# shubhamchandak94/HARC

Hardware: AMD Instinct MI355X
Metric: Mreads/s reorder+encode, 100 bp (higher is better)
Workload: dtype u64 (2-bit packed bases, XOR+popcount)

## Files before the change

### harc_amd/csrc/prims.hip

```cpp
#include "devutil.h"
#include <rocprim/rocprim.hpp>

int harc_tmp_reserve(harc_amd_ctx *c, size_t bytes)
{
    if (bytes <= c->tmp_bytes) return HARC_AMD_OK;
    if (c->d_tmp) harc_raw_free(c, c->d_tmp);
    c->d_tmp = nullptr; c->tmp_bytes = 0;
    size_t want = bytes + (bytes >> 3) + 4096;
    RC_TRY(harc_raw_alloc(c, &c->d_tmp, want));
    c->tmp_bytes = want;
    return HARC_AMD_OK;
}

#define PRIM_CALL(call_with_tmp)                                \
    do {                                                        \
        size_t bytes = 0; void *tmp = nullptr;                  \
        HIP_TRY(call_with_tmp);                                 \
        RC_TRY(harc_tmp_reserve(c, bytes));                     \
        tmp = c->d_tmp; bytes = c->tmp_bytes;                   \
        HIP_TRY(call_with_tmp);                                 \
    } while (0)

int prim_sort_pairs_u64_u32(harc_amd_ctx *c, const uint64_t *kin, uint64_t *kout, const uint32_t *vin, uint32_t *vout, size_t n, unsigned end_bit)
{
// ... 96 lines not shown
                M = __shfl(v, 63, 64);
            } else if (v > M) M = v;
            C += (uint32_t)__popcll(hb);
        }
    }
    if (!WRITE) {
        for (int o = 32; o > 0; o >>= 1) { const long long x = __shfl_xor(M, o, 64); if (x > M) M = x; }
        if (lane == 0) part[w] = BinPart{ M, C, 0u };
    }
}
int prim_bins_scan(harc_amd_ctx *c, const uint64_t *skeys, size_t n, uint64_t cap, uint32_t *binstart, uint64_t *q, uint32_t *nbins, void *scratch, size_t scratch_bytes)
{
    if (n == 0) return HARC_AMD_OK;
    const size_t room = scratch_bytes / (2 * sizeof(BinPart));
    if (room == 0 || n > 0xFFFFFFFFull || (n + room - 1) / room > (1u << 30) || room > 0x7FFFFFFFull) { harc_set_error("prim_bins_scan: %zu keys, scratch of %zu bytes", n, scratch_bytes); return HARC_AMD_EINVAL; }
    size_t seg = (n + room - 1) / room;
    if (seg < BINS_SEG_MIN) seg = BINS_SEG_MIN;
    seg = (seg + 64 * BINS_UNROLL - 1) / (64 * BINS_UNROLL) * (64 * BINS_UNROLL);
    const uint32_t nseg = (uint32_t)((n + seg - 1) / seg);
    BinPart *part = (BinPart *)scratch, *front = part + nseg;
    const dim3 grid((nseg + 3) / 4);
    hipLaunchKernelGGL(k_bins_pass<false>, grid, dim3(256), 0, c->stream, skeys, (uint32_t)n, cap, (uint32_t)seg, nseg, part, (uint32_t *)nullptr, (uint64_t *)nullptr, (uint32_t *)nullptr);
    PRIM_CALL(rocprim::exclusive_scan(tmp, bytes, part, front, BinPart{ BINS_NONE, 0u, 0u }, (size_t)nseg, BinPartOp(), c->stream));
    hipLaunchKernelGGL(k_bins_pass<true>, grid, dim3(256), 0, c->stream, skeys, (uint32_t)n, cap, (uint32_t)seg, nseg, front, binstart, q, nbins);
    HIP_TRY(hipGetLastError());
    return HARC_AMD_OK;
}

struct ContigPart { uint64_t s; uint32_t c, last; };
struct ContigPartOp {
    __host__ __device__ ContigPart operator()(const ContigPart &a, const ContigPart &b) const { return ContigPart{ a.s + b.s, a.c + b.c, a.last > b.last ? a.last : b.last }; }
};
#define CONTIG_SEG_MIN 2048u
#define CONTIG_SEGS 16384u
#define CONTIG_UNROLL 4
template <bool WRITE> __global__ __launch_bounds__(256) void k_contig_pass(const uint8_t *flag, const uint8_t *pos, uint32_t n, uint32_t L, uint32_t q, uint32_t cut, uint32_t seg, uint32_t nseg,
                                                                         ContigPart *part, uint8_t *head, uint32_t *cid, uint64_t *gstart, uint32_t *chead, unsigned long long *info)
{
    const uint32_t w = (blockIdx.x * 256u + threadIdx.x) >> 6;
    if (w >= nseg) return;
    const uint32_t lane = threadIdx.x & 63;
    const unsigned long long upto = ~0ull >> (63 - lane);
    uint32_t C = 0, last = 0; uint64_t G = 0;
    if (WRITE) { C = part[w].c; last = part[w].last; G = part[w].s; }
    const uint64_t base = (uint64_t)w * seg, end = base + seg < n ? base + seg : (uint64_t)n;
    uint32_t rem = (uint32_t)(base % q);
    for (uint64_t at = base; at < end; at += 64u * CONTIG_UNROLL) {
        uint8_t f[CONTIG_UNROLL], p[CONTIG_UNROLL];
#pragma unroll
        for (int u = 0; u < CONTIG_UNROLL; u++) { const uint64_t i = at + 64u * u + lane; f[u] = i < end ? flag[i] : (uint8_t)0; p[u] = i < end ? pos[i] : (uint8_t)0; }
#pragma unroll
        for (int u = 0; u < CONTIG_UNROLL; u++) {
            const uint64_t i0 = at + 64u * u, i = i0 + lane;
            const uint32_t m = rem + lane;
            const bool sh = q >= 128u ? (m == 0 || m == q) : (m % q) == 0;
            if (q >= 128u) { rem += 64u; if (rem >= q) rem -= q; } else rem = (rem + 64u) % q;
            const bool h = i < end && (f[u] == '0' || sh);
            const unsigned long long hb = __ballot(h);
            uint32_t v = i >= end ? 0u : h ? (i == 0 ? 0u : L) : (uint32_t)p[u];
            if (WRITE) {
                const uint32_t rank = C + (uint32_t)__popcll(hb & upto) - (h ? 1u : 0u);
                for (int d = 1; d < 64; d <<= 1) { const uint32_t o = __shfl_up(v, d, 64); if (lane >= (uint32_t)d) v += o; }
                const uint64_t g = G + v;
                const unsigned long long mine = hb & upto;
                const uint32_t l1 = mine ? (uint32_t)i0 + 63u - (uint32_t)__clzll(mine) : last;
                if (i < end) {
                    head[i] = h ? 1 : 0; cid[i] = rank; gstart[i] = g;
                    if (h) chead[rank] = (uint32_t)i;
                    if (sh) info[3 + (uint32_t)i / q] = g;
                    if ((uint32_t)i - l1 > cut) info[2] = 1;
                    if (i + 1 == n) { info[0] = rank + (h ? 1u : 0u); info[1] = g + L; }
                }
                G += __shfl(v, 63, 64);
            } else {
                for (int o = 32; o > 0; o >>= 1) v += __shfl_xor(v, o, 64);
                G += v;
            }
            if (hb) last = (uint32_t)i0 + 63u - (uint32_t)__clzll(hb);
            C += (uint32_t)__popcll(hb);
        }
    }
    if (!WRITE && lane == 0) part[w] = ContigPart{ G, C, last };
}
int prim_contig_scan(harc_amd_ctx *c, const uint8_t *flag, const uint8_t *pos, size_t n, uint32_t L, uint32_t q, uint32_t cut, uint8_t *head, uint32_t *cid, uint64_t *gstart,
                     uint32_t *chead, unsigned long long *info)
{
    if (n == 0) return HARC_AMD_OK;
    if (n > 0xFFFFFFFFull || q == 0) { harc_set_error("prim_contig_scan: %zu reads, shards of %u", n, q); return HARC_AMD_EINVAL; }
    size_t seg = (n + CONTIG_SEGS - 1) / CONTIG_SEGS;
    if (seg < CONTIG_SEG_MIN) seg = CONTIG_SEG_MIN;
    seg = (seg + 64 * CONTIG_UNROLL - 1) / (64 * CONTIG_UNROLL) * (64 * CONTIG_UNROLL);
    const uint32_t nseg = (uint32_t)((n + seg - 1) / seg);
    PoolScope scope(c);
    ContigPart *part = nullptr; RC_TRY(dalloc(c, &part, (size_t)2 * nseg));
    ContigPart *front = part + nseg;
    const dim3 grid((nseg + 3) / 4);
    HIP_TRY(hipMemsetAsync(info + 2, 0, 8, c->stream));
    hipLaunchKernelGGL(k_contig_pass<false>, grid, dim3(256), 0, c->stream, flag, pos, (uint32_t)n, L, q, cut, (uint32_t)seg, nseg, part, (uint8_t *)nullptr, (uint32_t *)nullptr, (uint64_t *)nullptr,
                       (uint32_t *)nullptr, (unsigned long long *)nullptr);
    PRIM_CALL(rocprim::exclusive_scan(tmp, bytes, part, front, ContigPart{ 0, 0u, 0u }, (size_t)nseg, ContigPartOp(), c->stream));
    hipLaunchKernelGGL(k_contig_pass<true>, grid, dim3(256), 0, c->stream, flag, pos, (uint32_t)n, L, q, cut, (uint32_t)seg, nseg, front, head, cid, gstart, chead, info);
    HIP_TRY(hipGetLastError());
    return HARC_AMD_OK;
}

__global__ void k_selftest_grid(uint64_t n, unsigned long long *out)
{
    const uint64_t i = harc_gid();
    unsigned long long one = i < n ? 1ULL : 0ULL, idx = i < n ? (unsigned long long)i : 0ULL;
    for (int o = 32; o > 0; o >>= 1) { one += __shfl_xor(one, o, 64); idx += __shfl_xor(idx, o, 64); }
    if ((threadIdx.x & 63) == 0 && one) { atomicAdd(&out[0], one); atomicAdd(&out[1], idx); }
}
__global__ void k_selftest_grid32(uint32_t n, unsigned long long *out)
{
    const uint32_t i = harc_gid32();
    unsigned long long one = i < n ? 1ULL : 0ULL, idx = i < n ? (unsigned long long)i : 0ULL;
    for (int o = 32; o > 0; o >>= 1) { one += __shfl_xor(one, o, 64); idx += __shfl_xor(idx, o, 64); }
    if ((threadIdx.x & 63) == 0 && one) { atomicAdd(&out[0], one); atomicAdd(&out[1], idx); }
}
__global__ void k_selftest_fold(uint64_t n, unsigned long long *out)
{
    const uint64_t wave = harc_bid() * 4 + (threadIdx.x >> 6);
    const int lane = threadIdx.x & 63;
    const uint64_t i = wave * 16 + (uint64_t)(lane >> 2);
    const bool mine = i < n && (lane & 3) == 0;
    unsigned long long one = mine ? 1ULL : 0ULL, idx = mine ? (unsigned long long)i : 0ULL;
    for (int o = 32; o > 0; o >>= 1) { one += __shfl_xor(one, o, 64); idx += __shfl_xor(idx, o, 64); }
    if (lane == 0 && one) { atomicAdd(&out[0], one); atomicAdd(&out[1], idx); }
}
extern "C" int harc_amd_selftest_launch(harc_amd_ctx *c, uint64_t n, uint64_t *visited, uint64_t *index_sum)
{
    if (!c || !visited || !index_sum) return HARC_AMD_EINVAL;
    HIP_TRY(hipSetDevice(c->P.device));
    unsigned long long *d = nullptr, h[6] = { 0, 0, 0, 0, 0, 0 };
    HIP_TRY(hipMalloc((void **)&d, sizeof h));
    const bool n32 = n <= 0xFFFFFFFFull;
    hipError_t e = hipMemsetAsync(d, 0, sizeof h, c->stream);
    if (e == hipSuccess) { hipLaunchKernelGGL(k_selftest_grid, harc_grid256(n), dim3(256), 0, c->stream, n, d); e = hipGetLastError(); }
    if (e == hipSuccess && n32) { hipLaunchKernelGGL(k_selftest_grid32, harc_grid256(n), dim3(256), 0, c->stream, (uint32_t)n, d + 2); e = hipGetLastError(); }
    if (e == hipSuccess) { hipLaunchKernelGGL(k_selftest_fold, harc_fold256((n + 63) / 64), dim3(256), 0, c->stream, n, d + 4); e = hipGetLastError(); }
    if (e == hipSuccess) e = hipMemcpyAsync(h, d, sizeof h, hipMemcpyDeviceToHost, c->stream);
    if (e == hipSuccess) e = hipStreamSynchronize(c->stream);
    (void)hipFree(d);
    if (e != hipSuccess) { harc_set_error("harc_amd_selftest_launch: %s", hipGetErrorString(e)); return HARC_AMD_ENODEVICE; }
    int k = 0;
    if (n32 && (h[2] != h[0] || h[3] != h[1])) k = 2;
    else if (h[4] != h[0] || h[5] != h[1]) k = 4;
    if (k) harc_set_error("harc_amd_selftest_launch: %s visited %llu items (index sum %llx), the thread-per-item grid %llu (%llx)", k == 2 ? "harc_gid32" : "harc_fold256 / harc_bid", h[k], h[k + 1], h[0], h[1]);
    *visited = h[k]; *index_sum = h[k + 1];
    return k ? HARC_AMD_EINTERNAL : HARC_AMD_OK;
}
```

### harc_amd/csrc/stage2.hip

```cpp
#include "devutil.h"
#include <time.h>
#include <algorithm>
#include <stdlib.h>

#define TUPLE_NONE 0xFFFFFFFFFFFFFFFFULL

struct S2Args {
    int L, W, W3, thresh_s, maxsearch;
    int ds[2], de[2], kbits[2];
    uint32_t M, S, T, q, nC;
    uint64_t total;
    const uint64_t *oreads;
    const uint64_t *reads;
    uint64_t *oreads_out;
    const uint8_t *flag, *pos, *rc;
    const uint32_t *order;
    const uint64_t *cand3;
    const uint32_t *cand_order;
    uint8_t *head;
    uint64_t *gstart;
    uint8_t *cons;
    const uint32_t *chead;
    const HashSlot *slots[2]; uint64_t cap[2]; const uint32_t *ids[2];
    unsigned long long *best;
// ... 1163 lines not shown
#define MERGE_TILE 2048
__global__ __launch_bounds__(256) void k_merge_orig(const uint64_t *gstart, uint32_t i0, uint32_t n, const uint64_t *tup, uint32_t A, FinalArrays f, uint32_t fbase, const long long *cut)
{
    __shared__ uint64_t cols[MERGE_TILE];
    const uint32_t t = harc_gid32();
    const long long c0 = cut[harc_bid()], c1 = cut[harc_bid() + 1] + 1;
    const long long inside = c1 - c0 - 1;
    const bool tiled = inside <= MERGE_TILE;
    if (tiled) {
        for (long long j = threadIdx.x; j < inside; j += 256) cols[j] = tup[c0 + 1 + j] >> 2;
        __syncthreads();
    }
    if (t >= n) return;
    const uint32_t i = i0 + t;
    const uint64_t g = gstart[i];
    long long lo = c0, hi = c1;
    if (tiled) while (hi - lo > 1) { const long long mid = (lo + hi) >> 1; if (cols[mid - c0 - 1] < g) lo = mid; else hi = mid; }
    else while (hi - lo > 1) { const long long mid = (lo + hi) >> 1; if ((tup[mid] >> 2) < g) lo = mid; else hi = mid; }
    const uint32_t at = i + (uint32_t)(lo + 1) - fbase;
    f.ref[at] = i; f.kind[at] = 0; f.g[at] = g;
}
__global__ void k_merge_acc(const uint64_t *gstart, uint32_t M, const uint64_t *tup, const uint32_t *rid, uint32_t a0, uint32_t na, FinalArrays f, uint32_t fbase)
{
    const uint32_t t = harc_gid32();
    if (t >= na) return;
    const uint32_t k = a0 + t;
    const uint64_t x = tup[k] >> 2;
    const long long n = ub_le(gstart, (long long)M, x) + 1;
    const uint32_t at = k + (uint32_t)n - fbase;
    f.ref[at] = rid[k]; f.kind[at] = (tup[k] & 2) ? 2 : 1; f.g[at] = x;
}
__global__ void k_shard_bounds(const uint64_t *gstart, uint32_t M, uint32_t q, uint32_t E, const uint64_t *tup, uint32_t A, uint64_t total, uint32_t *sh_f, uint32_t *sh_a, uint64_t *sh_col)
{
    const uint32_t e = harc_gid32();
    if (e > E) return;
    const uint64_t st = (uint64_t)e * q;
    if (e == E || st >= M) { sh_f[e] = M + A; sh_a[e] = A; sh_col[e] = total; return; }
    const uint64_t g = gstart[st];
    long long lo = -1, hi = A;
    while (hi - lo > 1) { const long long mid = (lo + hi) >> 1; if ((tup[mid] >> 2) < g) lo = mid; else hi = mid; }
    sh_f[e] = (uint32_t)st + (uint32_t)(lo + 1); sh_a[e] = (uint32_t)(lo + 1); sh_col[e] = g;
}

template <int W> __device__ __forceinline__ void final_words(const S2Args &s, uint32_t ref, int kind, uint64_t (&rd)[W], uint64_t (&nmk)[W])
{
    if (kind == 0) {
        const uint64_t *r = s.oreads + (size_t)ref * W;
#pragma unroll
        for (int w = 0; w < W; w++) { rd[w] = r[w]; nmk[w] = 0; }
        return;
    }
    constexpr int W3M = (3 * 32 * W + 63) / 64;
    uint64_t x3[W3M + 1];
    const uint64_t *r = s.cand3 + (size_t)ref * s.W3;
#pragma unroll
    for (int w = 0; w <= W3M; w++) x3[w] = w < s.W3 ? r[w] : 0;
    uint64_t a[W], n[W];
#pragma unroll
    for (int w = 0; w < W; w++) { a[w] = 0; n[w] = 0; }
#pragma unroll
    for (int j = 0; j < 32 * W; j++) {
        const int off = 3 * j, wi = off >> 6, sh = off & 63;
        uint64_t v = x3[wi] >> sh;
        if (sh > 61) v |= x3[wi + 1] << (64 - sh);
        const uint64_t c3 = v & 7;
        a[j >> 5] |= (c3 >> 1) << (2 * (j & 31));
        n[j >> 5] |= ((c3 & 1) * 3) << (2 * (j & 31));
    }
#pragma unroll
    for (int w = 0; w < W; w++) { const uint64_t lm = lowmask_word(2 * s.L, w); a[w] &= lm; n[w] &= lm; }
    if (kind == 1) {
#pragma unroll
        for (int w = 0; w < W; w++) { rd[w] = a[w]; nmk[w] = n[w]; }
    } else {
        uint64_t t[W];
        rc_words<W>(a, s.L, rd);
        rc_words<W>(n, s.L, t);
#pragma unroll
        for (int w = 0; w < W; w++) nmk[w] = ~t[w] & lowmask_word(2 * s.L, w);
    }
}
template <int W, bool EMIT> __global__ void k_noise(S2Args s, FinalArrays f, const uint64_t *cons2, uint32_t fb, uint32_t F, uint32_t *nm, uint32_t *nonN,
                                                    const uint64_t *nmoff, const uint32_t *nonNrank,
                                                    uint8_t *noise, uint8_t *noisepos, uint8_t *posb, uint8_t *rcb, uint32_t *order_out, uint32_t *orderN_out)
{
    const uint64_t i64 = (uint64_t)fb + harc_gid();
    if (i64 >= F) return;
    const uint32_t i = (uint32_t)i64;
    const uint32_t ref = f.ref[i]; const int kind = f.kind[i]; const uint64_t g = f.g[i];
    uint64_t rd[W], nk[W], cw[W], mm[W];
    final_words<W>(s, ref, kind, rd, nk);
    cons_words<W>(cons2, g, cw);
    uint32_t cnt = 0;
#pragma unroll
    for (int w = 0; w < W; w++) {
        const uint64_t x = rd[w] ^ cw[w];
        mm[w] = ((x | (x >> 1) | nk[w]) & 0x5555555555555555ULL) & lowmask_word(2 * s.L, w);
        cnt += (uint32_t)__popcll(mm[w]);
    }
    if (!EMIT) {
        nm[i] = cnt;
        nonN[i] = (kind != 0 && ref >= s.S) ? 0u : 1u;
        if (i + 1 == F) nm[F] = nonN[F] = 0;
        return;
    }
    uint64_t np = nmoff[i], nz = nmoff[i] + i;
    int prevj = 0;
#pragma unroll
    for (int w = 0; w < W; w++) {
        uint64_t m = mm[w];
        while (m) {
            const int b = __ffsll((long long)m) - 1; m &= m - 1;
            const int j = 32 * w + (b >> 1);
            const int rb = ((nk[w] >> b) & 1) ? 4 : pc_to_idx((int)((rd[w] >> b) & 3)), cb = pc_to_idx((int)((cw[w] >> b) & 3));
            noise[nz++] = (uint8_t)enc_noise(cb, rb); noisepos[np++] = (uint8_t)(j - prevj); prevj = j;
        }
    }
    noise[nz] = '\n';
    const bool is_head = (kind == 0) && s.head[ref];
    posb[i] = is_head ? (uint8_t)s.L : (uint8_t)(g - f.g[i - 1]);
    rcb[i] = kind == 0 ? s.rc[ref] : (kind == 1 ? 'd' : 'r');
    const uint32_t ov = kind == 0 ? s.order[ref] : s.cand_order[ref];
    const bool isN = (kind != 0 && ref >= s.S);
    if (isN) orderN_out[i - nonNrank[i]] = ov; else order_out[nonNrank[i]] = ov;
}
template <bool EMIT> static void launch_noise(harc_amd_ctx *c, const S2Args &a, const FinalArrays &f, const uint64_t *cons2, uint32_t fb, uint32_t F, uint32_t *nm, uint32_t *nonN,
                                              const uint64_t *nmoff, const uint32_t *nonNrank, uint8_t *noise, uint8_t *noisepos, uint8_t *posb, uint8_t *rcb,
                                              uint32_t *order_out, uint32_t *orderN_out)
{
#define NOISE_CASE(WW) case WW: hipLaunchKernelGGL((k_noise<WW, EMIT>), harc_grid256(F - fb), dim3(256), 0, c->stream, a, f, cons2, fb, F, nm, nonN, nmoff, nonNrank, noise, noisepos, posb, rcb, order_out, orderN_out); break;
    switch (a.W) { NOISE_CASE(1) NOISE_CASE(2) NOISE_CASE(3) NOISE_CASE(4) NOISE_CASE(5) NOISE_CASE(6) NOISE_CASE(7) NOISE_CASE(8) }
#undef NOISE_CASE
}

__global__ void k_left_flags(const unsigned long long *best, uint32_t t0, uint32_t n, uint32_t S, uint32_t *fs, uint32_t *fn)
{
    const uint32_t t = harc_gid32();
    if (t >= n) return;
    const uint32_t i = t0 + t;
    const bool un = best[i] == TUPLE_NONE;
    fs[t] = (un && i < S) ? 1u : 0u; fn[t] = (un && i >= S) ? 1u : 0u;
}
__global__ void k_left_orders(S2Args s, uint32_t t0, uint32_t nt, const uint32_t *rs, const uint32_t *rn, uint32_t *order_out, uint32_t order_base, uint32_t *orderN_out, uint32_t orderN_base)
{
    const uint32_t t = harc_gid32();
    if (t >= nt) return;
    const uint32_t i = t0 + t;
    if (s.best[i] != TUPLE_NONE) return;
    if (i < s.S) order_out[order_base + rs[t]] = s.cand_order[i]; else orderN_out[orderN_base + rn[t]] = s.cand_order[i];
}
__global__ void k_left_emit(S2Args s, uint32_t t0, uint32_t nt, const uint32_t *rs, const uint32_t *rn, uint8_t *sing_bases, char *ntext)
{
    const int G = (s.L + 15) / 16;
    const uint64_t gid = harc_gid();
    if (gid >= (uint64_t)nt * G) return;
    const uint32_t i = t0 + (uint32_t)(gid / G); const int g = (int)(gid % G);
    if (s.best[i] != TUPLE_NONE) return;
    const uint64_t *r = s.cand3 + (size_t)i * s.W3;
    const int j0 = 16 * g, j1 = j0 + 16 < s.L ? j0 + 16 : s.L;
    if (i < s.S) {
        const uint32_t k = rs[i - t0];
        uint8_t *o = sing_bases + (size_t)k * s.L;
        for (int j = j0; j < j1; j++) o[j] = (uint8_t)c3_to_idx5(c3_at(r, s.W3, j));
    } else {
        const uint32_t k = rn[i - t0];
        char *o = ntext + (size_t)k * (s.L + 1);
        for (int j = j0; j < j1; j++) o[j] = "ACGTN"[c3_to_idx5(c3_at(r, s.W3, j))];
        if (j1 == s.L) o[s.L] = '\n';
    }
}

__global__ void k_left_list(const uint32_t *fs, const uint32_t *fn, const uint32_t *rs, const uint32_t *rn, uint32_t nt, uint32_t US, uint32_t *list)
{
    const uint32_t t = harc_gid32();
    if (t >= nt) return;
    if (fs[t]) list[rs[t]] = t;
    else if (fn[t]) list[US + rn[t]] = t;
}
__global__ __launch_bounds__(256) void k_left_emit_w(S2Args s, uint32_t t0, const uint32_t *list, uint32_t nl, uint32_t US, uint8_t *sing_bases, char *ntext, uint32_t kbase)
{
    const uint32_t q = kbase + blockIdx.x * 4u + (threadIdx.x >> 6);
    const int lane = threadIdx.x & 63;
    if (q >= nl) return;
    const uint32_t i = t0 + list[q];
    const uint64_t *r = s.cand3 + (size_t)i * s.W3;
    const bool single = q < US;
    uint8_t *const ob = sing_bases + (size_t)q * s.L;
    char *const ot = ntext + (size_t)(q - US) * (s.L + 1);
    for (int j = lane; j < s.L; j += 64) {
        const int off = 3 * j, wi = off >> 6, sh = off & 63;
        const uint64_t lo = r[wi], hi = wi + 1 < s.W3 ? r[wi + 1] : 0ULL;
        const int c3 = (int)(((lo >> sh) | (sh ? (hi << (64 - sh)) : 0ULL)) & 7ULL);
        const int b = c3_to_idx5(c3);
        if (single) ob[j] = (uint8_t)b; else ot[j] = "ACGTN"[b];
    }
    if (!single && lane == 0) ot[s.L] = '\n';
}

struct SeqShard { uint64_t col0, nbytes, off; };
__global__ __launch_bounds__(256) void k_pack_seq(const uint64_t *cons2, const SeqShard *shards, uint8_t *out)
{
    const SeqShard sh = shards[blockIdx.y];
    const uint64_t j = (uint64_t)blockIdx.x * 256u + threadIdx.x;
    if (8 * j >= sh.nbytes) return;
    const uint64_t x = sh.col0 + 32 * j;
    const uint64_t *w = cons2 + (x >> 5);
    const int b = 2 * (int)(x & 31);
    uint64_t v = w[0] >> b;
    if (b) v |= w[1] << (64 - b);
    v = ((v & 0x5555555555555555ULL) << 1) | ((v >> 1) & 0x5555555555555555ULL);
    uint8_t *o = out + sh.off + 8 * j;
    if (8 * j + 8 <= sh.nbytes) *reinterpret_cast<uint64_t *>(o) = v;
    else for (uint64_t k = 0; 8 * j + k < sh.nbytes; k++) o[k] = (uint8_t)(v >> (8 * k));
// ... 511 lines not shown

    RC_TRY(best_digest("after the window passes"));
    lap("window passes over the large bins (all probes, on every rank)");
    unsigned long long big = 0;
    HIP_TRY(hipMemcpyAsync(&big, d_big, 8, hipMemcpyDeviceToHost, c->stream));
    HIP_TRY(hipStreamSynchronize(c->stream));
    ascope.release_now();
    const uint32_t nt = t1 - t0;
    uint32_t *ls = nullptr, *ln = nullptr, *rs = nullptr, *rn = nullptr;
    RC_TRY(dalloc(c, &ls, (size_t)nt + 1)); RC_TRY(dalloc(c, &ln, (size_t)nt + 1)); RC_TRY(dalloc(c, &rs, (size_t)nt + 1)); RC_TRY(dalloc(c, &rn, (size_t)nt + 1));
    HIP_TRY(hipMemsetAsync(ls, 0, ((size_t)nt + 1) * 4, c->stream)); HIP_TRY(hipMemsetAsync(ln, 0, ((size_t)nt + 1) * 4, c->stream));
    if (nt) hipLaunchKernelGGL(k_left_flags, G256(nt), best, t0, nt, S, ls, ln);
    RC_TRY(prim_excl_scan_u32(c, ls, rs, (size_t)nt + 1)); RC_TRY(prim_excl_scan_u32(c, ln, rn, (size_t)nt + 1));
    uint32_t US = 0, UN = 0;
    HIP_TRY(hipMemcpyAsync(&US, rs + nt, 4, hipMemcpyDeviceToHost, c->stream));
    HIP_TRY(hipMemcpyAsync(&UN, rn + nt, 4, hipMemcpyDeviceToHost, c->stream));
    HIP_TRY(hipStreamSynchronize(c->stream));
    uint8_t *sing_bases = nullptr, *spk = nullptr; char *ntext = nullptr;
    const uint64_t sing_nb = (uint64_t)US * L / 4, sing_tl = (uint64_t)US * L % 4;
    const size_t n_ntext = (size_t)UN * (L + 1);
    RC_TRY(dalloc(c, &sing_bases, (size_t)US * L + 8)); RC_TRY(dalloc(c, &ntext, n_ntext + 1)); RC_TRY(dalloc(c, &spk, (size_t)(sing_nb + sing_tl) + 64));
    uint8_t *h_sing = nullptr, *h_ntext = nullptr;
    RC_TRY(harc_host_alloc(c, (void **)&h_sing, (size_t)(sing_nb + sing_tl))); RC_TRY(harc_host_alloc(c, (void **)&h_ntext, n_ntext));
    if (getenv("HARC_AMD_LEFT_ALL")) { if (nt) hipLaunchKernelGGL(k_left_emit, G256((uint64_t)nt * ((L + 15) / 16)), a, t0, nt, rs, rn, sing_bases, ntext); }
    else if (US + UN) {
        uint32_t *llist = nullptr;
        RC_TRY(dalloc(c, &llist, (size_t)US + UN + 1));
        hipLaunchKernelGGL(k_left_list, G256(nt), (const uint32_t *)ls, (const uint32_t *)ln, (const uint32_t *)rs, (const uint32_t *)rn, nt, US, llist);
        WAVE_PER_ITEM(US + UN, hipLaunchKernelGGL(k_left_emit_w, dim3(nb_), dim3(256), 0, c->stream, a, t0, (const uint32_t *)llist, US + UN, US, sing_bases, ntext, kb_));
    }
    if (sing_nb) hipLaunchKernelGGL(k_pack2_bytes, G256(sing_nb), sing_bases, sing_nb, spk);
    if (sing_tl) hipLaunchKernelGGL(k_bases_to_ascii, G256(sing_tl), sing_bases + 4 * sing_nb, sing_tl, spk + sing_nb);
    HIP_TRY(hipGetLastError());
    HIP_TRY(hipEventRecord(c->ev_copy, c->stream));
    HIP_TRY(hipStreamWaitEvent(c->copy_stream, c->ev_copy, 0));
    if (sing_nb + sing_tl) HIP_TRY(hipMemcpyAsync(h_sing, spk, (size_t)(sing_nb + sing_tl), hipMemcpyDeviceToHost, c->copy_stream));
    if (n_ntext) HIP_TRY(hipMemcpyAsync(h_ntext, ntext, n_ntext, hipMemcpyDeviceToHost, c->copy_stream));
    uint32_t A = 0;
    uint32_t *ta = nullptr, *tb = nullptr; uint64_t *tup0 = nullptr, *tup = nullptr; uint32_t *rid0 = nullptr, *rid = nullptr;
    RC_TRY(dalloc(c, &ta, (size_t)T + 1)); RC_TRY(dalloc(c, &tb, (size_t)T + 1));
    if (T) {
        HIP_TRY(hipMemsetAsync(ta, 0, ((size_t)T + 1) * 4, c->stream));
        hipLaunchKernelGGL(k_acc_flags, G256(T), best, T, ta);
        RC_TRY(prim_excl_scan_u32(c, ta, tb, (size_t)T + 1));
        HIP_TRY(hipMemcpyAsync(&A, tb + T, 4, hipMemcpyDeviceToHost, c->stream));
        HIP_TRY(hipStreamSynchronize(c->stream));
    }
    RC_TRY(dalloc(c, &tup0, (size_t)A + 1)); RC_TRY(dalloc(c, &tup, (size_t)A + 1)); RC_TRY(dalloc(c, &rid0, (size_t)A + 1)); RC_TRY(dalloc(c, &rid, (size_t)A + 1));
    if (A) {
        hipLaunchKernelGGL(k_acc_compact, G256(T), best, tb, T, A, tup0, rid0);
        unsigned bits = 2; while (bits < 64 && (total >> (bits - 2)) != 0) bits++;
        RC_TRY(prim_sort_pairs_u64_u32(c, tup0, tup, rid0, rid, A, bits));
    }

    lap("accepted candidates sorted (all, on every rank)");
    std::vector<uint32_t> sh_f(E + 1), sh_a(E + 1);
    {
        uint32_t *d_shf = nullptr, *d_sha = nullptr; uint64_t *d_shc = nullptr;
        RC_TRY(dalloc(c, &d_shf, (size_t)E + 2)); RC_TRY(dalloc(c, &d_sha, (size_t)E + 2)); RC_TRY(dalloc(c, &d_shc, (size_t)E + 2));
        hipLaunchKernelGGL(k_shard_bounds, G256(E + 1), (const uint64_t *)gstart, M, a.q, E, (const uint64_t *)tup, A, total, d_shf, d_sha, d_shc);
        HIP_TRY(hipMemcpyAsync(sh_f.data(), d_shf, ((size_t)E + 1) * 4, hipMemcpyDeviceToHost, c->stream));
        HIP_TRY(hipMemcpyAsync(sh_a.data(), d_sha, ((size_t)E + 1) * 4, hipMemcpyDeviceToHost, c->stream));
        HIP_TRY(hipStreamSynchronize(c->stream));
    }
    const uint32_t fbase = sh_f[e0], fend = sh_f[e1], F = fend - fbase, na = sh_a[e1] - sh_a[e0];
    if ((uint64_t)(i1 - i0) + na != F) { harc_set_error("stage II bookkeeping: %u reads + %u accepted candidates in a piece of %u", i1 - i0, na, F); return HARC_AMD_EINTERNAL; }

    FinalArrays f;
    RC_TRY(dalloc(c, &f.ref, (size_t)F + 1)); RC_TRY(dalloc(c, &f.kind, (size_t)F + 1)); RC_TRY(dalloc(c, &f.g, (size_t)F + 1));
    uint32_t *nm = nullptr, *nonN = nullptr, *nonNrank = nullptr; uint64_t *nmoff = nullptr;
    RC_TRY(dalloc(c, &nm, (size_t)F + 1)); RC_TRY(dalloc(c, &nonN, (size_t)F + 1)); RC_TRY(dalloc(c, &nonNrank, (size_t)F + 1)); RC_TRY(dalloc(c, &nmoff, (size_t)F + 1));
    uint8_t *posb = nullptr, *rcb = nullptr;
    RC_TRY(dalloc(c, &posb, (size_t)F + 1)); RC_TRY(dalloc(c, &rcb, (size_t)F + 8));
    uint8_t *h_packed = nullptr, *h_pos = nullptr, *h_meta = nullptr;
    RC_TRY(harc_host_alloc(c, (void **)&h_pos, F)); RC_TRY(harc_host_alloc(c, (void **)&h_meta, 32));
    unsigned long long *h_tot = nullptr; RC_TRY(harc_host_alloc(c, (void **)&h_tot, 16 * ((size_t)E + 2)));
    std::vector<uint64_t> sh_nm(E + 1, 0);
    std::vector<uint8_t *> g_noise(E, nullptr), g_noisepos(E, nullptr), gh_noise(E, nullptr), gh_noisepos(E, nullptr);
    std::vector<uint32_t> g_of(E, 0);
    std::vector<uint64_t> gtot(E, 0);
    std::vector<uint64_t> s_nz0(E, 0), s_nz1(E, 0), s_np0(E, 0), s_np1(E, 0);
    long long *mcut = nullptr; RC_TRY(dalloc(c, &mcut, (size_t)(i1 - i0) / 256 + 4));
    uint64_t nmtot = 0; uint32_t n_nonN = 0, n_N_aligned = 0;
    const uint32_t estep = (uint64_t)F * 3 >= ((uint64_t)32 << 20) ? 1u : (e1 - e0 ? e1 - e0 : 1u);
    for (uint32_t ea = e0; ea < e1; ea += estep) {
        const uint32_t eb = ea + estep < e1 ? ea + estep : e1;
        for (uint32_t e = ea; e < eb; e++) g_of[e] = ea;
        const uint32_t fa = sh_f[ea] - fbase, fb = sh_f[eb] - fbase;
        if (fb <= fa) continue;
        const uint32_t ia = (uint32_t)((uint64_t)ea * a.q > M ? M : (uint64_t)ea * a.q), ib = eb >= E ? M : (uint32_t)((uint64_t)eb * a.q > M ? M : (uint64_t)eb * a.q);
        if (ib > ia) {
            hipLaunchKernelGGL(k_merge_cuts, G256((ib - ia + 255u) / 256u + 1u), gstart, ia, ib - ia, tup, A, mcut);
            hipLaunchKernelGGL(k_merge_orig, G256(ib - ia), gstart, ia, ib - ia, tup, A, f, fbase, (const long long *)mcut);
        }
        if (sh_a[eb] > sh_a[ea]) hipLaunchKernelGGL(k_merge_acc, G256(sh_a[eb] - sh_a[ea]), gstart, M, tup, rid, sh_a[ea], sh_a[eb] - sh_a[ea], f, fbase);
        launch_noise<false>(c, a, f, cons2, fa, fb, nm, nonN, nullptr, nullptr, nullptr, nullptr, nullptr, nullptr, nullptr, nullptr);
        RC_TRY(prim_excl_scan_u32_to_u64(c, nm + fa, nmoff + fa, (size_t)(fb - fa) + 1));
        RC_TRY(prim_excl_scan_u32(c, nonN + fa, nonNrank + fa, (size_t)(fb - fa) + 1));
        HIP_TRY(hipMemcpyAsync(&h_tot[0], nmoff + fb, 8, hipMemcpyDeviceToHost, c->stream));
        HIP_TRY(hipMemcpyAsync(reinterpret_cast<uint32_t *>(&h_tot[1]), nonNrank + fb, 4, hipMemcpyDeviceToHost, c->stream));
        for (uint32_t e = ea + 1; e < eb; e++) HIP_TRY(hipMemcpyAsync(&h_tot[2 + (e - ea)], nmoff + (sh_f[e] - fbase), 8, hipMemcpyDeviceToHost, c->stream));
        HIP_TRY(hipStreamSynchronize(c->stream));
        const uint64_t gnm = h_tot[0]; const uint32_t gnon = *reinterpret_cast<uint32_t *>(&h_tot[1]), gF = fb - fa;
        sh_nm[ea] = 0; for (uint32_t e = ea + 1; e < eb; e++) sh_nm[e] = h_tot[2 + (e - ea)];
        RC_TRY(dalloc(c, &g_noise[ea], (size_t)gnm + gF + 8)); RC_TRY(dalloc(c, &g_noisepos[ea], (size_t)gnm + 8));
        RC_TRY(harc_host_alloc(c, (void **)&gh_noise[ea], (size_t)gnm + gF)); RC_TRY(harc_host_alloc(c, (void **)&gh_noisepos[ea], (size_t)gnm));
        launch_noise<true>(c, a, f, cons2, fa, fb, nullptr, nullptr, nmoff, nonNrank, g_noise[ea] - fa, g_noisepos[ea], posb, rcb, order_out + n_nonN, orderN_out + n_N_aligned - fa);
        HIP_TRY(hipEventRecord(c->ev_copy, c->stream));
        HIP_TRY(hipStreamWaitEvent(c->copy_stream, c->ev_copy, 0));
        if (gnm + gF) HIP_TRY(hipMemcpyAsync(gh_noise[ea], g_noise[ea], (size_t)gnm + gF, hipMemcpyDeviceToHost, c->copy_stream));
        if (gnm) HIP_TRY(hipMemcpyAsync(gh_noisepos[ea], g_noisepos[ea], (size_t)gnm, hipMemcpyDeviceToHost, c->copy_stream));
        HIP_TRY(hipMemcpyAsync(h_pos + fa, posb + fa, (size_t)gF, hipMemcpyDeviceToHost, c->copy_stream));
        nmtot += gnm; n_nonN += gnon; n_N_aligned += gF - gnon;
        gtot[ea] = gnm;
        for (uint32_t e = ea; e < eb; e++) {
            const uint64_t n0 = sh_nm[e], n1 = e + 1 < eb ? sh_nm[e + 1] : gnm;
            s_np0[e] = n0; s_np1[e] = n1; s_nz0[e] = n0 + (sh_f[e] - sh_f[ea]); s_nz1[e] = n1 + (sh_f[e + 1] - sh_f[ea]);
        }
    }
    if ((size_t)n_nonN + US > (size_t)(i1 - i0) + (size_t)S || (size_t)n_N_aligned + UN > (size_t)NN) { harc_set_error("stage II bookkeeping: %u + %u clean, %u + %u N order entries", n_nonN, US, n_N_aligned, UN); return HARC_AMD_EINTERNAL; }
    const size_t n_order = ((size_t)n_nonN + US) * 4, n_orderN = ((size_t)n_N_aligned + UN) * 4;
    if (nt) hipLaunchKernelGGL(k_left_orders, G256(nt), a, t0, nt, rs, rn, order_out, n_nonN, orderN_out, n_N_aligned);
    HIP_TRY(hipGetLastError());
    if (c->d_gid && !c->s1_from_files) {
        unsigned int *d_merr = nullptr; RC_TRY(dalloc(c, &d_merr, 4));
        HIP_TRY(hipMemsetAsync(d_merr, 0, 16, c->stream));
        RC_TRY(shard_map_ids(c, order_out, (uint64_t)n_nonN + US, c->d_gid, c->N, d_merr));
        RC_TRY(shard_map_ids(c, orderN_out, (uint64_t)n_N_aligned + UN, c->d_ngid, c->NN, d_merr));
        unsigned int merr = 0;
        HIP_TRY(hipMemcpyAsync(&merr, d_merr, 4, hipMemcpyDeviceToHost, c->stream));
        HIP_TRY(hipStreamSynchronize(c->stream));
        if (merr) { harc_set_error("stage II: %u order entries outside the shard", merr); return HARC_AMD_EINTERNAL; }
    }

    std::vector<uint64_t> rev_off(E, 0), rev_nb(E, 0), rev_tl(E, 0);
    uint64_t poff = 0;
    for (uint32_t e = e0; e < e1; e++) {
        const uint64_t ff = sh_f[e + 1] - sh_f[e]; rev_nb[e] = ff / 8; rev_tl[e] = ff % 8; rev_off[e] = poff; poff += (rev_nb[e] + rev_tl[e] + 15) & ~15ull;
    }
    uint8_t *packed = nullptr; RC_TRY(dalloc(c, &packed, (size_t)poff + 64));
    for (uint32_t e = e0; e < e1; e++) {
        const uint32_t f0 = sh_f[e] - fbase;
        if (rev_nb[e]) hipLaunchKernelGGL(k_pack1_bytes, G256(rev_nb[e]), rcb + f0, rev_nb[e], packed + rev_off[e]);
        if (rev_tl[e]) HIP_TRY(hipMemcpyAsync(packed + rev_off[e] + rev_nb[e], rcb + f0 + 8 * rev_nb[e], rev_tl[e], hipMemcpyDeviceToDevice, c->stream));
    }
    HIP_TRY(hipGetLastError());
    RC_TRY(harc_host_alloc(c, (void **)&h_packed, (size_t)poff));
    HIP_TRY(hipEventRecord(c->ev_copy, c->stream));
    HIP_TRY(hipStreamWaitEvent(c->copy_stream, c->ev_copy, 0));
    if (poff) HIP_TRY(hipMemcpyAsync(h_packed, packed, (size_t)poff, hipMemcpyDeviceToHost, c->copy_stream));
    if (want_digest) {
        for (uint32_t e = e0; e < e1; e++) if (g_of[e] == e && g_noise[e]) {
            uint32_t eb = e; while (eb < e1 && g_of[eb] == e) eb++;
            RC_TRY(digest_range(c, g_noise[e], gtot[e] + (sh_f[eb] - sh_f[e]), 0x200 + 16 * e, d_digest + 1)); RC_TRY(digest_range(c, g_noisepos[e], gtot[e], 0x201 + 16 * e, d_digest + 1));
        }
        RC_TRY(digest_range(c, posb, F, 0x202, d_digest + 1));
        for (uint32_t e = e0; e < e1; e++) RC_TRY(digest_range(c, packed + rev_off[e], rev_nb[e] + rev_tl[e], 0x300 + e, d_digest + 2));
        RC_TRY(digest_range(c, spk, sing_nb + sing_tl, 0x3F0, d_digest + 2)); RC_TRY(digest_range(c, ntext, n_ntext, 0x3F1, d_digest + 2));
        RC_TRY(digest_range(c, order_out, n_order, 0x400, d_digest + 3)); RC_TRY(digest_range(c, orderN_out, n_orderN, 0x401, d_digest + 3));
        unsigned long long *h_dig = nullptr; RC_TRY(harc_host_alloc(c, (void **)&h_dig, 32));
        HIP_TRY(hipMemcpyAsync(h_dig, d_digest, 32, hipMemcpyDeviceToHost, c->stream));
        HIP_TRY(hipStreamSynchronize(c->stream));
        for (int k = 0; k < 4; k++) c->digest[k] = h_dig[k];
        for (uint32_t e = e0; e <= e1; e++) { c->digest[1] += mix64(0x2F0ull + e + ((uint64_t)(sh_f[e] - fbase) << 20)) + (e < e1 ? mix64(0x2F8ull + e + (s_np1[e] << 20)) : 0ull); c->digest[0] += mix64(0x1F0ull + e + ((sh_col[e] - col0) << 20)); }
        c->have_digest = true;
    }
    for (uint32_t e = 0; e < E; e++) {
        if (e < e0 || e >= e1) {
            for (int id : { HARC_AMD_S2_SEQ, HARC_AMD_S2_SEQ_TAIL, HARC_AMD_S2_REV, HARC_AMD_S2_REV_TAIL, HARC_AMD_S2_POS, HARC_AMD_S2_NOISE, HARC_AMD_S2_NOISEPOS }) out_slice(c, id, e, h_meta, 0);
            continue;
        }
        const uint32_t f0 = sh_f[e] - fbase, f1 = sh_f[e + 1] - fbase;
        out_slice(c, HARC_AMD_S2_SEQ, e, h_seq + seq_off[e], seq_nb[e]); out_slice(c, HARC_AMD_S2_SEQ_TAIL, e, h_seq + seq_off[e] + seq_nb[e], seq_tl[e]);
        out_slice(c, HARC_AMD_S2_REV, e, h_packed + rev_off[e], rev_nb[e]); out_slice(c, HARC_AMD_S2_REV_TAIL, e, h_packed + rev_off[e] + rev_nb[e], rev_tl[e]);
        out_slice(c, HARC_AMD_S2_POS, e, h_pos + f0, f1 - f0);
        const uint32_t g = g_of[e];
        out_slice(c, HARC_AMD_S2_NOISE, e, gh_noise[g] ? gh_noise[g] + s_nz0[e] : h_meta, gh_noise[g] ? s_nz1[e] - s_nz0[e] : 0);
        out_slice(c, HARC_AMD_S2_NOISEPOS, e, gh_noisepos[g] ? gh_noisepos[g] + s_np0[e] : h_meta, gh_noisepos[g] ? s_np1[e] - s_np0[e] : 0);
    }
    out_slice(c, HARC_AMD_S2_SINGLETON, 0, h_sing, sing_nb); out_slice(c, HARC_AMD_S2_SINGLETON_TAIL, 0, h_sing + sing_nb, sing_tl);
    c->d_s2_order = order_out; c->n_s2_order = n_order; c->d_s2_orderN = orderN_out; c->n_s2_orderN = n_orderN;
    out_slice(c, HARC_AMD_S2_INPUT_N, 0, h_ntext, n_ntext);
    { const int ml = snprintf((char *)h_meta, 32, "%d\n", L); out_slice(c, HARC_AMD_S2_META, 0, h_meta, (size_t)ml); }
    HIP_TRY(hipStreamSynchronize(c->stream));
    HIP_TRY(hipStreamSynchronize(c->copy_stream));
    if (trace2) fprintf(stderr, "[stage II] %llu noise entries, %u reads in this rank's piece\n", (unsigned long long)nmtot, F);
    lap("merge, noise / pos / rev / order streams, leftovers, device -> host (this rank's shards)");
    c->C.bins_over_maxsearch = big;
    const uint32_t s_lo = t0 < S ? t0 : S, s_hi = t1 < S ? t1 : S;
    c->C.aligned_singletons = (uint64_t)(s_hi - s_lo) - US;
// ... 32 lines not shown
```

Baseline: 791.4.

## Vectorize contig scan to four reads per lane and skip zero-noise word work

Adds a contig-scan kernel variant where each lane handles four consecutive reads. It uses 32-bit loads of flag/pos and vector stores of head/cid/gstart, and does one warp scan per 256 reads instead of per 64. The old kernel stays as a fallback for misaligned pointers or when an env var is set. The noise emit kernel now reads the precomputed mismatch offsets and skips rebuilding read and consensus words for reads with no mismatches. This trades extra per-lane registers and an extra nmoff load for fewer instructions and narrower memory traffic.

```diff
diff --git a/harc_amd/csrc/prims.hip b/harc_amd/csrc/prims.hip
--- a/harc_amd/csrc/prims.hip
+++ b/harc_amd/csrc/prims.hip
@@ -202,6 +202,94 @@
     }
     if (!WRITE && lane == 0) part[w] = ContigPart{ G, C, last };
 }
+template <bool WRITE> __global__ __launch_bounds__(256) void k_contig_pass4(const uint8_t *flag, const uint8_t *pos, uint32_t n, uint32_t L, uint32_t q, uint32_t cut, uint32_t seg, uint32_t nseg,
+                                                                          ContigPart *part, uint8_t *head, uint32_t *cid, uint64_t *gstart, uint32_t *chead, unsigned long long *info)
+{
+    const uint32_t w = (blockIdx.x * 256u + threadIdx.x) >> 6;
+    if (w >= nseg) return;
+    const uint32_t lane = threadIdx.x & 63;
+    const unsigned long long below = (1ull << lane) - 1;
+    uint32_t C = 0, last = 0; uint64_t G = 0;
+    if (WRITE) { C = part[w].c; last = part[w].last; G = part[w].s; }
+    const uint64_t base = (uint64_t)w * seg, end = base + seg < n ? base + seg : (uint64_t)n;
+    uint32_t rem = (uint32_t)(base % q);
+    for (uint64_t at = base; at < end; at += 256u * CONTIG_UNROLL) {
+        uint32_t f4[CONTIG_UNROLL], p4[CONTIG_UNROLL];
+#pragma unroll
+        for (int u = 0; u < CONTIG_UNROLL; u++) {
+            const uint64_t i4 = at + 256u * u + 4u * lane;
+            if (i4 + 4 <= end) { f4[u] = *reinterpret_cast<const uint32_t *>(flag + i4); p4[u] = *reinterpret_cast<const uint32_t *>(pos + i4); }
+            else {
+                f4[u] = p4[u] = 0;
+#pragma unroll
+                for (int k = 0; k < 4; k++) if (i4 + k < end) { f4[u] |= (uint32_t)flag[i4 + k] << (8 * k); p4[u] |= (uint32_t)pos[i4 + k] << (8 * k); }
+            }
+        }
+#pragma unroll
+        for (int u = 0; u < CONTIG_UNROLL; u++) {
+            const uint64_t i0 = at + 256u * u, i4 = i0 + 4u * lane;
+            bool h[4], sh[4]; unsigned long long hb[4]; uint32_t v[4];
+#pragma unroll
+            for (int k = 0; k < 4; k++) {
+                const uint64_t i = i4 + k;
+                const uint32_t m = rem + 4u * lane + k;
+                sh[k] = q >= 256u ? (m == 0 || m == q) : (m % q) == 0;
+                h[k] = i < end && (((f4[u] >> (8 * k)) & 255u) == '0' || sh[k]);
+                hb[k] = __ballot(h[k]);
+                v[k] = i >= end ? 0u : h[k] ? (i == 0 ? 0u : L) : ((p4[u] >> (8 * k)) & 255u);
+            }
+            if (q >= 256u) { rem += 256u; if (rem >= q) rem -= q; } else rem = (rem + 256u) % q;
+            uint32_t trip_last = last; bool any = false;
+#pragma unroll
+            for (int k = 0; k < 4; k++) if (hb[k]) { const uint32_t x = (uint32_t)i0 + 4u * (63u - (uint32_t)__clzll(hb[k])) + k; if (!any || x > trip_last) trip_last = x; any = true; }
+            const uint32_t heads = (uint32_t)(__popcll(hb[0]) + __popcll(hb[1]) + __popcll(hb[2]) + __popcll(hb[3]));
+            uint32_t t = v[0] + v[1] + v[2] + v[3];
+            if (WRITE) {
+                uint32_t rank = C + (uint32_t)(__popcll(hb[0] & below) + __popcll(hb[1] & below) + __popcll(hb[2] & below) + __popcll(hb[3] & below));
+                uint32_t l1 = last; bool lower = false;
+#pragma unroll
+                for (int k = 0; k < 4; k++) {
+                    const unsigned long long b = hb[k] & below;
+                    if (b) { const uint32_t x = (uint32_t)i0 + 4u * (63u - (uint32_t)__clzll(b)) + k; if (!lower || x > l1) l1 = x; lower = true; }
+                }
+                uint32_t incl = t;
+                for (int d = 1; d < 64; d <<= 1) { const uint32_t o = __shfl_up(incl, d, 64); if (lane >= (uint32_t)d) incl += o; }
+                uint64_t g = G + (incl - t);
+                uint32_t r4[4]; uint64_t g4[4]; bool far = false;
+#pragma unroll
+                for (int k = 0; k < 4; k++) {
+                    const uint64_t i = i4 + k;
+                    g += v[k]; g4[k] = g; r4[k] = rank;
+                    if (h[k]) l1 = (uint32_t)i;
+                    if (i < end) {
+                        if (h[k]) chead[rank] = (uint32_t)i;
+                        if (sh[k]) info[3 + (uint32_t)i / q] = g;
+                        if ((uint32_t)i - l1 > cut) far = true;
+                        if (i + 1 == n) { info[0] = rank + (h[k] ? 1u : 0u); info[1] = g + L; }
+                    }
+                    rank += h[k] ? 1u : 0u;
+                }
+                if (far) info[2] = 1;
+                if (i4 + 4 <= end) {
+                    *reinterpret_cast<uint32_t *>(head + i4) = (h[0] ? 1u : 0u) | (h[1] ? 1u << 8 : 0u) | (h[2] ? 1u << 16 : 0u) | (h[3] ? 1u << 24 : 0u);
+                    *reinterpret_cast<uint4 *>(cid + i4) = make_uint4(r4[0], r4[1], r4[2], r4[3]);
+                    *reinterpret_cast<ulonglong2 *>(gstart + i4) = make_ulonglong2(g4[0], g4[1]);
+                    *reinterpret_cast<ulonglong2 *>(gstart + i4 + 2) = make_ulonglong2(g4[2], g4[3]);
+                } else {
+#pragma unroll
+                    for (int k = 0; k < 4; k++) if (i4 + k < end) { head[i4 + k] = h[k] ? 1 : 0; cid[i4 + k] = r4[k]; gstart[i4 + k] = g4[k]; }
+                }
+                G += __shfl(incl, 63, 64);
+            } else {
+                for (int o = 32; o > 0; o >>= 1) t += __shfl_xor(t, o, 64);
+                G += t;
+            }
+            last = trip_last;
+            C += heads;
+        }
+    }
+    if (!WRITE && lane == 0) part[w] = ContigPart{ G, C, last };
+}
 int prim_contig_scan(harc_amd_ctx *c, const uint8_t *flag, const uint8_t *pos, size_t n, uint32_t L, uint32_t q, uint32_t cut, uint8_t *head, uint32_t *cid, uint64_t *gstart,
                      uint32_t *chead, unsigned long long *info)
 {
@@ -209,17 +297,19 @@
     if (n > 0xFFFFFFFFull || q == 0) { harc_set_error("prim_contig_scan: %zu reads, shards of %u", n, q); return HARC_AMD_EINVAL; }
     size_t seg = (n + CONTIG_SEGS - 1) / CONTIG_SEGS;
     if (seg < CONTIG_SEG_MIN) seg = CONTIG_SEG_MIN;
-    seg = (seg + 64 * CONTIG_UNROLL - 1) / (64 * CONTIG_UNROLL) * (64 * CONTIG_UNROLL);
+    const bool one = (getenv("HARC_AMD_S2_CONTIG1") && atoi(getenv("HARC_AMD_S2_CONTIG1")) != 0) || (((uintptr_t)flag | (uintptr_t)pos | (uintptr_t)head) & 3) || (((uintptr_t)cid | (uintptr_t)gstart) & 15);
+    const size_t trips = (one ? 64 : 256) * CONTIG_UNROLL;
+    seg = (seg + trips - 1) / trips * trips;
     const uint32_t nseg = (uint32_t)((n + seg - 1) / seg);
     PoolScope scope(c);
     ContigPart *part = nullptr; RC_TRY(dalloc(c, &part, (size_t)2 * nseg));
     ContigPart *front = part + nseg;
     const dim3 grid((nseg + 3) / 4);
     HIP_TRY(hipMemsetAsync(info + 2, 0, 8, c->stream));
-    hipLaunchKernelGGL(k_contig_pass<false>, grid, dim3(256), 0, c->stream, flag, pos, (uint32_t)n, L, q, cut, (uint32_t)seg, nseg, part, (uint8_t *)nullptr, (uint32_t *)nullptr, (uint64_t *)nullptr,
-                       (uint32_t *)nullptr, (unsigned long long *)nullptr);
+    hipLaunchKernelGGL(one ? k_contig_pass<false> : k_contig_pass4<false>, grid, dim3(256), 0, c->stream, flag, pos, (uint32_t)n, L, q, cut, (uint32_t)seg, nseg, part, (uint8_t *)nullptr, (uint32_t *)nullptr,
+                       (uint64_t *)nullptr, (uint32_t *)nullptr, (unsigned long long *)nullptr);
     PRIM_CALL(rocprim::exclusive_scan(tmp, bytes, part, front, ContigPart{ 0, 0u, 0u }, (size_t)nseg, ContigPartOp(), c->stream));
-    hipLaunchKernelGGL(k_contig_pass<true>, grid, dim3(256), 0, c->stream, flag, pos, (uint32_t)n, L, q, cut, (uint32_t)seg, nseg, front, head, cid, gstart, chead, info);
+    hipLaunchKernelGGL(one ? k_contig_pass<true> : k_contig_pass4<true>, grid, dim3(256), 0, c->stream, flag, pos, (uint32_t)n, L, q, cut, (uint32_t)seg, nseg, front, head, cid, gstart, chead, info);
     HIP_TRY(hipGetLastError());
     return HARC_AMD_OK;
 }
diff --git a/harc_amd/csrc/stage2.hip b/harc_amd/csrc/stage2.hip
--- a/harc_amd/csrc/stage2.hip
+++ b/harc_amd/csrc/stage2.hip
@@ -1269,53 +1269,63 @@
 }
 template <int W, bool EMIT> __global__ void k_noise(S2Args s, FinalArrays f, const uint64_t *cons2, uint32_t fb, uint32_t F, uint32_t *nm, uint32_t *nonN,
                                                     const uint64_t *nmoff, const uint32_t *nonNrank,
-                                                    uint8_t *noise, uint8_t *noisepos, uint8_t *posb, uint8_t *rcb, uint32_t *order_out, uint32_t *orderN_out)
+                                                    uint8_t *noise, uint8_t *noisepos, uint8_t *posb, uint8_t *rcb, uint32_t *order_out, uint32_t *orderN_out, int emit_all)
 {
     const uint64_t i64 = (uint64_t)fb + harc_gid();
     if (i64 >= F) return;
     const uint32_t i = (uint32_t)i64;
     const uint32_t ref = f.ref[i]; const int kind = f.kind[i]; const uint64_t g = f.g[i];
-    uint64_t rd[W], nk[W], cw[W], mm[W];
-    final_words<W>(s, ref, kind, rd, nk);
-    cons_words<W>(cons2, g, cw);
-    uint32_t cnt = 0;
-#pragma unroll
-    for (int w = 0; w < W; w++) {
-        const uint64_t x = rd[w] ^ cw[w];
-        mm[w] = ((x | (x >> 1) | nk[w]) & 0x5555555555555555ULL) & lowmask_word(2 * s.L, w);
-        cnt += (uint32_t)__popcll(mm[w]);
-    }
-    if (!EMIT) {
-        nm[i] = cnt;
-        nonN[i] = (kind != 0 && ref >= s.S) ? 0u : 1u;
-        if (i + 1 == F) nm[F] = nonN[F] = 0;
-        return;
-    }
-    uint64_t np = nmoff[i], nz = nmoff[i] + i;
-    int prevj = 0;
-#pragma unroll
-    for (int w = 0; w < W; w++) {
-        uint64_t m = mm[w];
-        while (m) {
-            const int b = __ffsll((long long)m) - 1; m &= m - 1;
-            const int j = 32 * w + (b >> 1);
-            const int rb = ((nk[w] >> b) & 1) ? 4 : pc_to_idx((int)((rd[w] >> b) & 3)), cb = pc_to_idx((int)((cw[w] >> b) & 3));
-            noise[nz++] = (uint8_t)enc_noise(cb, rb); noisepos[np++] = (uint8_t)(j - prevj); prevj = j;
+    uint64_t np = 0, nz = 0;
+    bool words = true, is_head = false, isN = false; uint8_t rcv = 0; uint32_t ov = 0, nr = 0; uint64_t gprev = 0;
+    if (EMIT) {
+        np = nmoff[i]; nz = np + i;
+        words = emit_all || nmoff[i + 1] != np;
+        is_head = (kind == 0) && s.head[ref];
+        gprev = i > 0 ? f.g[i - 1] : 0;
+        rcv = kind == 0 ? s.rc[ref] : (kind == 1 ? 'd' : 'r');
+        ov = kind == 0 ? s.order[ref] : s.cand_order[ref];
+        isN = (kind != 0 && ref >= s.S);
+        nr = nonNrank[i];
+    }
+    if (words) {
+        uint64_t rd[W], nk[W], cw[W], mm[W];
+        final_words<W>(s, ref, kind, rd, nk);
+        cons_words<W>(cons2, g, cw);
+        uint32_t cnt = 0;
+#pragma unroll
+        for (int w = 0; w < W; w++) {
+            const uint64_t x = rd[w] ^ cw[w];
+            mm[w] = ((x | (x >> 1) | nk[w]) & 0x5555555555555555ULL) & lowmask_word(2 * s.L, w);
+            cnt += (uint32_t)__popcll(mm[w]);
+        }
+        if (!EMIT) {
+            nm[i] = cnt;
+            nonN[i] = (kind != 0 && ref >= s.S) ? 0u : 1u;
+            if (i + 1 == F) nm[F] = nonN[F] = 0;
+            return;
+        }
+        int prevj = 0;
+#pragma unroll
+        for (int w = 0; w < W; w++) {
+            uint64_t m = mm[w];
+            while (m) {
+                const int b = __ffsll((long long)m) - 1; m &= m - 1;
+                const int j = 32 * w + (b >> 1);
+                const int rb = ((nk[w] >> b) & 1) ? 4 : pc_to_idx((int)((rd[w] >> b) & 3)), cb = pc_to_idx((int)((cw[w] >> b) & 3));
+                noise[nz++] = (uint8_t)enc_noise(cb, rb); noisepos[np++] = (uint8_t)(j - prevj); prevj = j;
+            }
         }
     }
     noise[nz] = '\n';
-    const bool is_head = (kind == 0) && s.head[ref];
-    posb[i] = is_head ? (uint8_t)s.L : (uint8_t)(g - f.g[i - 1]);
-    rcb[i] = kind == 0 ? s.rc[ref] : (kind == 1 ? 'd' : 'r');
-    const uint32_t ov = kind == 0 ? s.order[ref] : s.cand_order[ref];
-    const bool isN = (kind != 0 && ref >= s.S);
-    if (isN) orderN_out[i - nonNrank[i]] = ov; else order_out[nonNrank[i]] = ov;
+    posb[i] = is_head ? (uint8_t)s.L : (uint8_t)(g - gprev);
+    rcb[i] = rcv;
+    if (isN) orderN_out[i - nr] = ov; else order_out[nr] = ov;
 }
 template <bool EMIT> static void launch_noise(harc_amd_ctx *c, const S2Args &a, const FinalArrays &f, const uint64_t *cons2, uint32_t fb, uint32_t F, uint32_t *nm, uint32_t *nonN,
                                               const uint64_t *nmoff, const uint32_t *nonNrank, uint8_t *noise, uint8_t *noisepos, uint8_t *posb, uint8_t *rcb,
-                                              uint32_t *order_out, uint32_t *orderN_out)
-{
-#define NOISE_CASE(WW) case WW: hipLaunchKernelGGL((k_noise<WW, EMIT>), harc_grid256(F - fb), dim3(256), 0, c->stream, a, f, cons2, fb, F, nm, nonN, nmoff, nonNrank, noise, noisepos, posb, rcb, order_out, orderN_out); break;
+                                              uint32_t *order_out, uint32_t *orderN_out, int emit_all = 0)
+{
+#define NOISE_CASE(WW) case WW: hipLaunchKernelGGL((k_noise<WW, EMIT>), harc_grid256(F - fb), dim3(256), 0, c->stream, a, f, cons2, fb, F, nm, nonN, nmoff, nonNrank, noise, noisepos, posb, rcb, order_out, orderN_out, emit_all); break;
     switch (a.W) { NOISE_CASE(1) NOISE_CASE(2) NOISE_CASE(3) NOISE_CASE(4) NOISE_CASE(5) NOISE_CASE(6) NOISE_CASE(7) NOISE_CASE(8) }
 #undef NOISE_CASE
 }
@@ -1993,6 +2003,7 @@
     std::vector<uint64_t> s_nz0(E, 0), s_nz1(E, 0), s_np0(E, 0), s_np1(E, 0);
     long long *mcut = nullptr; RC_TRY(dalloc(c, &mcut, (size_t)(i1 - i0) / 256 + 4));
     uint64_t nmtot = 0; uint32_t n_nonN = 0, n_N_aligned = 0;
+    const int emit_all = getenv("HARC_AMD_S2_EMIT_ALL") && atoi(getenv("HARC_AMD_S2_EMIT_ALL")) != 0;
     const uint32_t estep = (uint64_t)F * 3 >= ((uint64_t)32 << 20) ? 1u : (e1 - e0 ? e1 - e0 : 1u);
     for (uint32_t ea = e0; ea < e1; ea += estep) {
         const uint32_t eb = ea + estep < e1 ? ea + estep : e1;
@@ -2016,7 +2027,7 @@
         sh_nm[ea] = 0; for (uint32_t e = ea + 1; e < eb; e++) sh_nm[e] = h_tot[2 + (e - ea)];
         RC_TRY(dalloc(c, &g_noise[ea], (size_t)gnm + gF + 8)); RC_TRY(dalloc(c, &g_noisepos[ea], (size_t)gnm + 8));
         RC_TRY(harc_host_alloc(c, (void **)&gh_noise[ea], (size_t)gnm + gF)); RC_TRY(harc_host_alloc(c, (void **)&gh_noisepos[ea], (size_t)gnm));
-        launch_noise<true>(c, a, f, cons2, fa, fb, nullptr, nullptr, nmoff, nonNrank, g_noise[ea] - fa, g_noisepos[ea], posb, rcb, order_out + n_nonN, orderN_out + n_N_aligned - fa);
+        launch_noise<true>(c, a, f, cons2, fa, fb, nullptr, nullptr, nmoff, nonNrank, g_noise[ea] - fa, g_noisepos[ea], posb, rcb, order_out + n_nonN, orderN_out + n_N_aligned - fa, emit_all);
         HIP_TRY(hipEventRecord(c->ev_copy, c->stream));
         HIP_TRY(hipStreamWaitEvent(c->copy_stream, c->ev_copy, 0));
         if (gnm + gF) HIP_TRY(hipMemcpyAsync(gh_noise[ea], g_noise[ea], (size_t)gnm + gF, hipMemcpyDeviceToHost, c->copy_stream));
```

Result: no change. 795.9, median of 6 (+0.6%).
